# KadAMRN/Data_Free_Quantization

Hardware: AMD Instinct MI355X
Metric: weight-GB/s quantized (per-ch INT8 DFQ sweep) + top-1 delta, MobileNetV2 (higher is better)
Workload: dtype f32

## Files before the change

data_free_quantization_amd/csrc/dfq_transform.hip:

```cpp
#include "dfq_common.h"

#include <cstdlib>
#include <cstring>

#include <algorithm>
#include <chrono>
#include <cmath>
#include <mutex>
#include <new>
#include <string>
#include <vector>

namespace dfq {

static int blocks_for(int64_t n, int per_thread = 1) {
    const int64_t b = ceil_div(std::max<int64_t>(n, 1), (int64_t)kThreads * per_thread);
    return (int)std::min<int64_t>(b, 256 * 8);
}

__device__ __forceinline__ float bn_factor(float g, float v, float eps) {
    return g / sqrtf(v + eps);
}

__global__ void bn_fold_weight_kernel(float* __restrict__ w, const float* __restrict__ g,
                                      const float* __restrict__ v, float eps, int64_t rows, int64_t len) {
    const int64_t n = rows * len;
    for (int64_t i = (int64_t)blockIdx.x * blockDim.x + threadIdx.x; i < n; i += (int64_t)gridDim.x * blockDim.x) {
        const int64_t o = i / len;
        w[i] = w[i] * bn_factor(g[o], v[o], eps);
    }
}

__global__ void bn_fold_channel_kernel(float* __restrict__ bias, float* __restrict__ g, float* __restrict__ b,
                                       float* __restrict__ m, float* __restrict__ v, float* __restrict__ fake_w,
                                       float* __restrict__ fake_b, float eps, int64_t rows) {
    for (int64_t o = (int64_t)blockIdx.x * blockDim.x + threadIdx.x; o < rows; o += (int64_t)gridDim.x * blockDim.x) {
        const float go = g[o], bo = b[o], mo = m[o], vo = v[o];
        const float f = bn_factor(go, vo, eps);
        const float shift = bo - (go * mo) / sqrtf(vo + eps);
        bias[o] = bias[o] * f + shift;
        if (fake_w) fake_w[o] = fabsf(go);
        if (fake_b) fake_b[o] = bo;
        g[o] = 1.0f;
        v[o] = 1.0f;
        b[o] = 0.0f;
        m[o] = 0.0f;
    }
}

__global__ void clamp_kernel(float* __restrict__ w, int64_t n, float lo, float hi) {
    const int64_t n4 = n >> 2;
    float4* w4 = reinterpret_cast<float4*>(w);
    for (int64_t i = (int64_t)blockIdx.x * blockDim.x + threadIdx.x; i < n4; i += (int64_t)gridDim.x * blockDim.x) {
        float4 v = w4[i];
        v.x = fminf(fmaxf(v.x, lo), hi);
        v.y = fminf(fmaxf(v.y, lo), hi);
        v.z = fminf(fmaxf(v.z, lo), hi);
        v.w = fminf(fmaxf(v.w, lo), hi);
        w4[i] = v;
    }
    for (int64_t i = 4 * n4 + (int64_t)blockIdx.x * blockDim.x + threadIdx.x; i < n; i += (int64_t)gridDim.x * blockDim.x)
        w[i] = fminf(fmaxf(w[i], lo), hi);
}

__device__ __forceinline__ float absorb_c(float beta, float gamma, float n_sigma) {
    float c = beta - n_sigma * gamma;
    return (c < 0.0f) ? 0.0f : c;
}

__global__ void absorb_gemv_kernel(const float* __restrict__ w2, float* __restrict__ b2,
                                   const float* __restrict__ bn_w, const float* __restrict__ bn_b,
                                   int64_t o2, int64_t i2, int64_t khw2, int64_t o2g, float n_sigma) {
    const int lane = threadIdx.x & 63;
    const int64_t wave = (int64_t)blockIdx.x * (blockDim.x / 64) + (threadIdx.x >> 6);
    const int64_t nwaves = (int64_t)gridDim.x * (blockDim.x / 64);
    for (int64_t o = wave; o < o2; o += nwaves) {
        const int64_t g = o / o2g;
        const float* row = w2 + o * i2 * khw2;
        float acc = 0.f;
        for (int64_t i = lane; i < i2; i += 64) {
            float ssum = 0.f;
            for (int64_t k = 0; k < khw2; ++k) ssum += row[i * khw2 + k];
            const int64_t ch = g * i2 + i;
            acc += ssum * absorb_c(bn_b[ch], bn_w[ch], n_sigma);
        }
        acc = wave_sum_f(acc);
        if (lane == 0) b2[o] = b2[o] + acc;
    }
}

__global__ void absorb_channel_kernel(float* __restrict__ b1, float* __restrict__ bn_b, const float* __restrict__ bn_w,
                                      int64_t c1, float n_sigma) {
    for (int64_t c = (int64_t)blockIdx.x * blockDim.x + threadIdx.x; c < c1; c += (int64_t)gridDim.x * blockDim.x) {
        const float cc = absorb_c(bn_b[c], bn_w[c], n_sigma);
        b1[c] = b1[c] + (-cc);
        bn_b[c] = bn_b[c] + (-cc);
    }
}

__device__ __forceinline__ double ndtr_d(double a) {
    const double x = a * 0.70710678118654752440;
    const double z = fabs(x);
    if (z < 0.70710678118654752440) return 0.5 + 0.5 * erf(x);
    const double y = 0.5 * erfc(z);
    return x > 0.0 ? 1.0 - y : y;
}

__device__ __forceinline__ float bc_expect_value(float wj, float bj, int relu) {
    if (!relu) return bj;
    const float x = (-bj) / wj;
    const double xd = (double)x;
    const float pdf = (float)(exp(-(xd * xd) / 2.0) / 2.5066282746310002);
    const float cdf = (float)ndtr_d(xd);
    float ex = wj * pdf + bj * (1.0f - cdf);
    if (ex < 0.0f) ex = 0.0f;
    return ex;
}

__global__ void bc_expect_kernel(const float* __restrict__ w, const float* __restrict__ b, int64_t n, int relu,
                                 int accumulate, float* __restrict__ out) {
    for (int64_t j = (int64_t)blockIdx.x * blockDim.x + threadIdx.x; j < n; j += (int64_t)gridDim.x * blockDim.x) {
        const float ex = bc_expect_value(w[j], b[j], relu);
        out[j] = accumulate ? out[j] + ex : ex;
    }
}

__global__ void __launch_bounds__(kThreads)
bc_apply_kernel(const float* __restrict__ E, int64_t o, int64_t i2, const float* __restrict__ ex, int64_t f,
                int64_t bcols, float* __restrict__ bias, float* __restrict__ bias_vec) {
    const int lane = threadIdx.x & 63;
    const int64_t wave = (int64_t)blockIdx.x * (kThreads / 64) + (threadIdx.x >> 6);
    const int64_t nwaves = (int64_t)gridDim.x * (kThreads / 64);
    for (int64_t r = wave; r < o; r += nwaves) {
        auto get = [&](int64_t j) { return E[r * i2 + (i2 > 1 ? j : 0)] + ex[f > 1 ? j : 0]; };
        if (bias_vec)
            for (int64_t j = lane; j < bcols; j += 64) bias_vec[r * bcols + j] = get(j);
        const float sum = wave_inner_sum(get, bcols, lane);
        if (lane == 0) bias[r] = bias[r] + sum / (float)bcols;
    }
}

constexpr int64_t kBcScratch = 1024;
__global__ void __launch_bounds__(kThreads)
bc_propagate_kernel(const float* __restrict__ bias_vec, int64_t nrows, int64_t f, int threads,
                    float* __restrict__ fake_b) {
    __shared__ float scratch[kThreads / 64][kBcScratch + kBcScratch / 16];
    const int lane = threadIdx.x & 63;
    const int wv = threadIdx.x >> 6;
    float* b0s = scratch[wv];
    float* b1s = b0s + kBcScratch;
    const int64_t wave = (int64_t)blockIdx.x * (kThreads / 64) + wv;
    const int64_t nwaves = (int64_t)gridDim.x * (kThreads / 64);
    for (int64_t c = wave; c < f; c += nwaves) {
        auto get = [&](int64_t r) { return bias_vec[r * f + c]; };
        const float sum = aten_outer_col_is_cascade(nrows, f, c, threads)
                              ? wave_cascade(get, nrows, lane, b0s, b1s, kBcScratch)
                              : wave_row_sum(get, nrows, lane, b0s, b1s, kBcScratch);
        if (lane == 0) fake_b[c] = fake_b[c] + (-sum) / (float)nrows;
    }
}



constexpr int kBcMaxTerms = 8;
constexpr int64_t kBcMaxExpect = 4096;
struct BcLayerJob {
    const float* ew[kBcMaxTerms];
    const float* eb[kBcMaxTerms];
    int32_t relu[kBcMaxTerms];
    int32_t nterms;
    int32_t threads;
    float* expect_out;
    int64_t f;
    const float* E;
    int64_t o, i2, bcols;
    float* bias;
    float* vec;
    float* fake_b;
    int64_t F, nrows;
    int64_t apply_blocks;
};

constexpr int64_t kBcStage = 2048;
__global__ void __launch_bounds__(kThreads) bc_layer_kernel(BcLayerJob J) {
    __shared__ float ex[kBcMaxExpect];
    __shared__ float scratch[kThreads / 64][kBcScratch + kBcScratch / 16];
    __shared__ float stage[kThreads / 64][kBcStage];
    for (int64_t j = threadIdx.x; j < J.f; j += kThreads) {
        float v = bc_expect_value(J.ew[0][j], J.eb[0][j], J.relu[0]);
        for (int t = 1; t < J.nterms; ++t) v = v + bc_expect_value(J.ew[t][j], J.eb[t][j], J.relu[t]);
        ex[j] = v;
        if (blockIdx.x == 0) J.expect_out[j] = v;
    }
    __syncthreads();
    const int lane = threadIdx.x & 63;
    const int wv = threadIdx.x >> 6;
    const bool ebc = J.i2 > 1, xbc = J.f > 1;
    if ((int64_t)blockIdx.x < J.apply_blocks) {
        const int64_t wave = (int64_t)blockIdx.x * (kThreads / 64) + wv;
        const int64_t nwaves = J.apply_blocks * (kThreads / 64);
        float* rowv = stage[wv];
        for (int64_t r = wave; r < J.o; r += nwaves) {
            auto get = [&](int64_t j) { return J.E[r * J.i2 + (ebc ? j : 0)] + ex[xbc ? j : 0]; };
            for (int64_t j = lane; j < J.bcols; j += 64) {
                const float v = get(j);
                rowv[j] = v;
                if (J.vec) J.vec[r * J.bcols + j] = v;
            }
            wave_lds_sync();
            const float sum = wave_inner_sum([&](int64_t j) { return rowv[j]; }, J.bcols, lane);
            wave_lds_sync();
            if (lane == 0) J.bias[r] = J.bias[r] + sum / (float)J.bcols;
        }
        return;
    }
    float* b0s = scratch[wv];
    float* b1s = b0s + kBcScratch;
    const int64_t wave = ((int64_t)blockIdx.x - J.apply_blocks) * (kThreads / 64) + wv;
    const int64_t nwaves = ((int64_t)gridDim.x - J.apply_blocks) * (kThreads / 64);
    float* colv = stage[wv];
    for (int64_t c = wave; c < J.F; c += nwaves) {
        auto get = [&](int64_t r) {
            const uint32_t idx = (uint32_t)r * (uint32_t)J.F + (uint32_t)c;
            const uint32_t row = idx / (uint32_t)J.bcols, j = idx - row * (uint32_t)J.bcols;
            return J.E[(int64_t)row * J.i2 + (ebc ? j : 0)] + ex[xbc ? j : 0];
        };
        const bool cascade = aten_outer_col_is_cascade(J.nrows, J.F, c, J.threads);
        for (int64_t r = lane; r < J.nrows; r += 64) colv[r] = get(r);
        wave_lds_sync();
        auto lds = [&](int64_t r) { return colv[r]; };
        const float sum = cascade ? wave_cascade(lds, J.nrows, lane, b0s, b1s, kBcScratch)
                                  : wave_row_sum(lds, J.nrows, lane, b0s, b1s, kBcScratch);
        wave_lds_sync();
        if (lane == 0) J.fake_b[c] = J.fake_b[c] + (-sum) / (float)J.nrows;
    }
}

__device__ __forceinline__ float std_pdf(float x) {
    const double xd = (double)x;
    return (float)(exp(-(xd * xd) / 2.0) / 2.5066282746310002);
}
__device__ __forceinline__ float std_cdf(float x) { return (float)ndtr_d((double)x); }

__global__ void act_moments_kernel(const float* w_in, const float* b_in, int64_t n, int kind, int sqrt_w, float eps,
                                   int accumulate, float* mean, float* var) {
    for (int64_t j = (int64_t)blockIdx.x * blockDim.x + threadIdx.x; j < n; j += (int64_t)gridDim.x * blockDim.x) {
        const float w = sqrt_w ? sqrtf(w_in[j] + eps) : w_in[j];
        const float b = b_in[j];
        float m, v;
        if (kind == 0) {
            m = b;
            v = w * w;
        } else if (kind == 1) {
            const float x0 = (-b) / w;
            const float P0 = std_pdf(x0), C0 = std_cdf(x0);
            m = w * P0 + b * (1.0f - C0);
            const float B = ((b * b + w * w) + m * m) - (2.0f * m) * b;
            v = ((1.0f - C0) * B + (w * (b - 2.0f * m)) * P0) + (m * m) * C0;
        } else {
            const float x0 = (-b) / w, x6 = (6.0f - b) / w;
            const float P0 = std_pdf(x0), C0 = std_cdf(x0), P6 = std_pdf(x6), C6 = std_cdf(x6);
            m = (w * (P0 - P6) + b * (C6 - C0)) + 6.0f * (1.0f - C6);
            const float B = ((b * b + w * w) + m * m) - (2.0f * m) * b;
            const float d6 = 6.0f - m;
            v = ((((C6 - C0) * B + (w * -6.0f) * P6) + (w * (b - 2.0f * m)) * (P0 - P6)) + (m * m) * C0) +
                (d6 * d6) * (1.0f - C6);
        }
        if (accumulate) {
            m = mean[j] + m;
            v = var[j] + v;
        }
        mean[j] = m;
        var[j] = v;
    }
}

__global__ void act_minmax_kernel(const float* a, const float* w_in, int64_t n, int w_is_var, float eps, float nsig,
                                  float* out) {
    __shared__ float smin[4], smax[4];
    float vmin = INFINITY, vmax = -INFINITY;
    for (int64_t j = threadIdx.x; j < n; j += blockDim.x) {
        const float w = w_is_var ? sqrtf(w_in[j] + eps) : w_in[j];
        const float nw = nsig * w;
        vmin = fminf(vmin, a[j] - nw);
        vmax = fmaxf(vmax, a[j] + nw);
    }
    vmin = wave_min(vmin);
    vmax = wave_max(vmax);
    if ((threadIdx.x & 63) == 0) {
        smin[threadIdx.x >> 6] = vmin;
        smax[threadIdx.x >> 6] = vmax;
    }
    __syncthreads();
    if (threadIdx.x == 0) {
        for (int k = 1; k < (int)(blockDim.x / 64); ++k) {
            vmin = fminf(vmin, smin[k]);
            vmax = fmaxf(vmax, smax[k]);
        }
        out[0] = fminf(smin[0], vmin);
        out[1] = fmaxf(smax[0], vmax);
    }
}

__global__ void act_affine_kernel(const float* x, const float* w, const float* bias, int64_t o, int64_t i2,
                                  int64_t khw, int64_t og, float* out) {
    const int lane = threadIdx.x & 63;
    const int64_t wave = (int64_t)blockIdx.x * (blockDim.x / 64) + (threadIdx.x >> 6);
    const int64_t nwaves = (int64_t)gridDim.x * (blockDim.x / 64);
    for (int64_t r = wave; r < o; r += nwaves) {
        const int64_t g = r / og;
        float acc = 0.f;
        for (int64_t i = lane; i < i2; i += 64) {
            const float* p = w + (r * i2 + i) * khw;
            const float ws = khw == 1 ? p[0] : aten_inner_sum([&](int64_t k) { return p[k]; }, khw);
            acc += ws * x[g * i2 + i];
        }
        acc = wave_sum_f(acc);
        if (lane == 0) out[r] = bias ? acc + bias[r] : acc;
    }
}


struct BnFoldJob {
    float* w;
    float* bias;
    float* g;
    float* b;
    float* m;
    float* v;
    float* fake_w;
    float* fake_b;
    float eps;
    int32_t flags;
    int64_t rows, row_len;
    uint32_t* range_enc;
};
struct BnFoldChunk {
    int32_t job;
    int32_t pad;
    int64_t e0, e1;
};

__device__ __forceinline__ float fold_factor(const BnFoldJob& J, int64_t o) {
    const float go = ((const DFQ_GLOBAL float*)J.g)[o], ve = ((const DFQ_GLOBAL float*)J.v)[o] + J.eps;
    return (go == 1.0f && ve == 1.0f) ? 1.0f : go / sqrtf(ve);
}

__device__ __forceinline__ int64_t fold_row(const BnFoldJob& J, int64_t r0, int64_t base, float inv, int64_t i,
                                            int* rem_out) {
    const int li = (int)(i - base);
    const int len = (int)J.row_len;
    int q = (int)((float)li * inv);
    int rem = li - q * len;
    if (rem < 0) {
        --q;
        rem += len;
    } else if (rem >= len) {
        ++q;
        rem -= len;
    }
    *rem_out = rem;
    return r0 + q;
}

__device__ __forceinline__ float fold_one(const BnFoldJob& J, int64_t r0, int64_t base, float inv, int64_t i,
                                          float w) {
    int rem;
    const float f = fold_factor(J, fold_row(J, r0, base, inv, i, &rem));
    return f != 1.0f ? w * f : w;
}

__global__ void __launch_bounds__(kThreads)
bn_fold_weight_batch_kernel(const BnFoldJob* __restrict__ jobs, const BnFoldChunk* __restrict__ chunks,
                            int64_t nchunks) {
    __shared__ float smn[kThreads / kWave], smx[kThreads / kWave];
    for (int64_t c = blockIdx.x; c < nchunks; c += gridDim.x) {
        const BnFoldChunk ch = chunks[c];
        const BnFoldJob J = jobs[ch.job];
        const int64_t r0 = ch.e0 / J.row_len, base = r0 * J.row_len;
        const float inv = 1.0f / (float)J.row_len;
        float a = INFINITY, b = -INFINITY;
        const int64_t n = ch.e1 - ch.e0;
        int64_t done = 0;
        int ident = 1;
        for (int64_t r = r0 + threadIdx.x; r <= (ch.e1 - 1) / J.row_len; r += blockDim.x)
            ident &= fold_factor(J, r) == 1.0f;
        ident = __syncthreads_and(ident);
        if (ident && (reinterpret_cast<uintptr_t>(J.w + ch.e0) & 15) == 0) {
            const DFQ_GLOBAL f32x4* w4 = (const DFQ_GLOBAL f32x4*)(J.w + ch.e0);
            const int64_t n4 = n >> 2;
            for (int64_t k = threadIdx.x; k < n4; k += 4 * (int64_t)blockDim.x) {
                f32x4 v[4];
#pragma unroll
                for (int u = 0; u < 4; ++u)
                    if (k + u * (int64_t)blockDim.x < n4) v[u] = w4[k + u * blockDim.x];
#pragma unroll
                for (int u = 0; u < 4; ++u)
                    if (k + u * (int64_t)blockDim.x < n4) {
                        a = fminf(a, fminf(fminf(v[u].x, v[u].y), fminf(v[u].z, v[u].w)));
                        b = fmaxf(b, fmaxf(fmaxf(v[u].x, v[u].y), fmaxf(v[u].z, v[u].w)));
                    }
            }
            done = 4 * n4;
        } else if ((reinterpret_cast<uintptr_t>(J.w + ch.e0) & 15) == 0) {
            DFQ_GLOBAL f32x4* w4 = (DFQ_GLOBAL f32x4*)(J.w + ch.e0);
            const int64_t n4 = n >> 2;
            for (int64_t k = threadIdx.x; k < n4; k += blockDim.x) {
                const f32x4 v = w4[k];
                const int64_t i = ch.e0 + 4 * k;
                f32x4 o;
                int rem;
                const float f = fold_factor(J, fold_row(J, r0, base, inv, i, &rem));
                if (rem + 3 < (int)J.row_len) {
                    o.x = f != 1.0f ? v.x * f : v.x;
                    o.y = f != 1.0f ? v.y * f : v.y;
                    o.z = f != 1.0f ? v.z * f : v.z;
                    o.w = f != 1.0f ? v.w * f : v.w;
                } else {
                    o.x = f != 1.0f ? v.x * f : v.x;
                    o.y = fold_one(J, r0, base, inv, i + 1, v.y);
                    o.z = fold_one(J, r0, base, inv, i + 2, v.z);
                    o.w = fold_one(J, r0, base, inv, i + 3, v.w);
                }
                if (__float_as_uint(o.x) != __float_as_uint(v.x) || __float_as_uint(o.y) != __float_as_uint(v.y) ||
                    __float_as_uint(o.z) != __float_as_uint(v.z) || __float_as_uint(o.w) != __float_as_uint(v.w))
                    w4[k] = o;
                a = fminf(a, fminf(fminf(o.x, o.y), fminf(o.z, o.w)));
                b = fmaxf(b, fmaxf(fmaxf(o.x, o.y), fmaxf(o.z, o.w)));
            }
            done = 4 * n4;
        }
        DFQ_GLOBAL float* wg = (DFQ_GLOBAL float*)J.w;
        for (int64_t k = done + threadIdx.x; k < n; k += blockDim.x) {
            const int64_t i = ch.e0 + k;
            const float v = wg[i];
            const float o = fold_one(J, r0, base, inv, i, v);
            if (__float_as_uint(o) != __float_as_uint(v)) wg[i] = o;
            a = fminf(a, o);
            b = fmaxf(b, o);
        }
        if (J.range_enc) {
            a = wave_min(a);
            b = wave_max(b);
            const int lane = threadIdx.x & (kWave - 1), wv = threadIdx.x >> 6;
            if (lane == 0) {
                smn[wv] = a;
                smx[wv] = b;
            }
            __syncthreads();
            if (threadIdx.x == 0) {
                for (int k = 1; k < kThreads / kWave; ++k) {
                    a = fminf(a, smn[k]);
                    b = fmaxf(b, smx[k]);
                }
                atomicMax(&J.range_enc[0], ~enc_ord(a));
                atomicMax(&J.range_enc[1], enc_ord(b));
            }
            __syncthreads();
        }
    }
}

__global__ void bn_fold_channel_batch_kernel(const BnFoldJob* __restrict__ jobs, int32_t njobs) {
    for (int32_t j = blockIdx.x; j < njobs; j += gridDim.x) {
        const BnFoldJob J = jobs[j];
        typedef DFQ_GLOBAL float* G;
        const G g = (G)J.g, b = (G)J.b, m = (G)J.m, v = (G)J.v, bias = (G)J.bias, fw = (G)J.fake_w, fb = (G)J.fake_b;
        for (int64_t o = threadIdx.x; o < J.rows; o += blockDim.x) {
            const float go = g[o], bo = b[o], mo = m[o], vo = v[o];
            const float f = bn_factor(go, vo, J.eps);
            const float shift = bo - (go * mo) / sqrtf(vo + J.eps);
            const float b0 = (J.flags & DFQ_BN_FOLD_ZERO_BIAS) ? 0.0f : bias[o];
            bias[o] = b0 * f + shift;
            if (J.fake_w) fw[o] = fabsf(go);
            if (J.fake_b) fb[o] = bo;
            g[o] = 1.0f;
            v[o] = 1.0f;
            b[o] = 0.0f;
            m[o] = 0.0f;
        }
    }
}

__device__ __forceinline__ float qdq_nan(float x, const QParams& p, float& q) {
    const float y = qdq(x, p, q);
    return x != x ? x : y;
}

__global__ void __launch_bounds__(kThreads)
fq_given_kernel(const float* __restrict__ x, float* __restrict__ y, int64_t n, int bits, int sym, int flags,
                const float* __restrict__ min_dev, const float* __restrict__ max_dev,
                const uint32_t* __restrict__ range_enc, double gmin, double gmax, int vec4) {
    if (min_dev) gmin = (double)min_dev[0];
    if (max_dev) gmax = (double)max_dev[0];
    if (range_enc) {
        gmin = (double)dec_ord(~range_enc[0]);
        gmax = (double)dec_ord(range_enc[1]);
    }
    const QParams p = make_qparams((float)gmin, (float)gmax, bits, sym != 0, flags | DFQ_GIVEN_RANGE, gmin, gmax);
    const int64_t stride = (int64_t)gridDim.x * blockDim.x;
    float q;
    if (vec4) {
        const int64_t n4 = n >> 2;
        for (int64_t i = (int64_t)blockIdx.x * blockDim.x + threadIdx.x; i < n4; i += stride) {
            const float4 v = reinterpret_cast<const float4*>(x)[i];
            float4 o;
            o.x = qdq_nan(v.x, p, q);
            o.y = qdq_nan(v.y, p, q);
            o.z = qdq_nan(v.z, p, q);
            o.w = qdq_nan(v.w, p, q);
            reinterpret_cast<float4*>(y)[i] = o;
        }
    } else {
        for (int64_t i = (int64_t)blockIdx.x * blockDim.x + threadIdx.x; i < n; i += stride)
            y[i] = qdq_nan(x[i], p, q);
    }
}

constexpr int64_t kFqSmall = 16384;

__global__ void __launch_bounds__(kThreads)
fq_tensor_small_kernel(const float* __restrict__ x, float* __restrict__ y, int64_t n, int bits, int sym, int flags) {
    __shared__ float smn[kThreads / kWave], smx[kThreads / kWave];
    float a = INFINITY, b = -INFINITY;
    for (int64_t i = threadIdx.x; i < n; i += kThreads) {
        const float v = x[i];
        a = fminf(a, v);
        b = fmaxf(b, v);
    }
    a = wave_min(a);
    b = wave_max(b);
    const int lane = threadIdx.x & (kWave - 1), w = threadIdx.x >> 6;
    if (lane == 0) {
        smn[w] = a;
        smx[w] = b;
    }
    __syncthreads();
// ... 908 lines not shown
```

Before: 1859.

## Prefetch first bias-correction row/column into LDS during expectation compute

Before the expectation computation, each wave in the bias-correction kernel issues asynchronous global-to-LDS loads for its first row or column of E, plus an early load of the old bias value. The loads then overlap with the expectation loop and are waited on before the barrier. The first loop iteration reads the prefetched LDS values instead of global memory. This aims to hide global load latency, at the cost of more complex control flow and reliance on the global_load_lds intrinsic and its waitcnt encoding.

```diff
diff --git a/data_free_quantization_amd/csrc/dfq_transform.hip b/data_free_quantization_amd/csrc/dfq_transform.hip
--- a/data_free_quantization_amd/csrc/dfq_transform.hip
+++ b/data_free_quantization_amd/csrc/dfq_transform.hip
@@ -182,57 +182,92 @@
 };
 
 constexpr int64_t kBcStage = 2048;
+#ifndef DFQ_BC_PREFETCH
+#define DFQ_BC_PREFETCH 1
+#endif
 __global__ void __launch_bounds__(kThreads) bc_layer_kernel(BcLayerJob J) {
     __shared__ float ex[kBcMaxExpect];
     __shared__ float scratch[kThreads / 64][kBcScratch + kBcScratch / 16];
     __shared__ float stage[kThreads / 64][kBcStage];
+    const int lane = threadIdx.x & 63;
+    const int wv = wave_uniform(threadIdx.x >> 6);
+    const bool ebc = J.i2 > 1, xbc = J.f > 1;
+    const bool apply = (int64_t)blockIdx.x < J.apply_blocks;
+    const int64_t wave = ((int64_t)blockIdx.x - (apply ? 0 : J.apply_blocks)) * (kThreads / 64) + wv;
+    const int64_t nwaves = (apply ? J.apply_blocks : (int64_t)gridDim.x - J.apply_blocks) * (kThreads / 64);
+    auto gather = [&](int64_t r, int64_t c, uint32_t& j) {
+        const uint32_t idx = (uint32_t)r * (uint32_t)J.F + (uint32_t)c;
+        const uint32_t row = idx / (uint32_t)J.bcols;
+        j = idx - row * (uint32_t)J.bcols;
+        return (int64_t)row * J.i2 + (ebc ? j : 0);
+    };
+#if DFQ_BC_PREFETCH
+    float old = 0.f;
+    const bool have = wave < (apply ? J.o : J.F);
+    const int n0 = have ? (int)(apply ? J.bcols : J.nrows) : 0;
+    DFQ_LDS float* slot = (DFQ_LDS float*)stage[wv];
+    for (int k = 0; 64 * k < n0; ++k) {
+        const int e = min(lane + 64 * k, n0 - 1);
+        uint32_t j;
+        const float* src = J.E + (apply ? wave * J.i2 + (ebc ? e : 0) : gather(e, wave, j));
+        __builtin_amdgcn_global_load_lds((const DFQ_GLOBAL void*)src, (DFQ_LDS void*)(slot + 64 * k), 4, 0, 0);
+    }
+    const float* oldp = (apply ? J.bias : J.fake_b) + (have ? wave : 0);
+    if (have && lane == 0) old = *oldp;
+    bool first = true;
+#else
+    const float old = 0.f;
+    const bool first = false;
+#endif
     for (int64_t j = threadIdx.x; j < J.f; j += kThreads) {
         float v = bc_expect_value(J.ew[0][j], J.eb[0][j], J.relu[0]);
         for (int t = 1; t < J.nterms; ++t) v = v + bc_expect_value(J.ew[t][j], J.eb[t][j], J.relu[t]);
         ex[j] = v;
         if (blockIdx.x == 0) J.expect_out[j] = v;
     }
+#if DFQ_BC_PREFETCH
+    __builtin_amdgcn_s_waitcnt(0x0F70);
+#endif
     __syncthreads();
-    const int lane = threadIdx.x & 63;
-    const int wv = threadIdx.x >> 6;
-    const bool ebc = J.i2 > 1, xbc = J.f > 1;
-    if ((int64_t)blockIdx.x < J.apply_blocks) {
-        const int64_t wave = (int64_t)blockIdx.x * (kThreads / 64) + wv;
-        const int64_t nwaves = J.apply_blocks * (kThreads / 64);
+    if (apply) {
         float* rowv = stage[wv];
         for (int64_t r = wave; r < J.o; r += nwaves) {
-            auto get = [&](int64_t j) { return J.E[r * J.i2 + (ebc ? j : 0)] + ex[xbc ? j : 0]; };
             for (int64_t j = lane; j < J.bcols; j += 64) {
-                const float v = get(j);
+                const float e = first ? rowv[j] : J.E[r * J.i2 + (ebc ? j : 0)];
+                const float v = e + ex[xbc ? j : 0];
                 rowv[j] = v;
                 if (J.vec) J.vec[r * J.bcols + j] = v;
             }
             wave_lds_sync();
             const float sum = wave_inner_sum([&](int64_t j) { return rowv[j]; }, J.bcols, lane);
             wave_lds_sync();
-            if (lane == 0) J.bias[r] = J.bias[r] + sum / (float)J.bcols;
+            if (lane == 0) J.bias[r] = (first ? old : J.bias[r]) + sum / (float)J.bcols;
+#if DFQ_BC_PREFETCH
+            first = false;
+#endif
         }
         return;
     }
     float* b0s = scratch[wv];
     float* b1s = b0s + kBcScratch;
-    const int64_t wave = ((int64_t)blockIdx.x - J.apply_blocks) * (kThreads / 64) + wv;
-    const int64_t nwaves = ((int64_t)gridDim.x - J.apply_blocks) * (kThreads / 64);
     float* colv = stage[wv];
     for (int64_t c = wave; c < J.F; c += nwaves) {
-        auto get = [&](int64_t r) {
-            const uint32_t idx = (uint32_t)r * (uint32_t)J.F + (uint32_t)c;
-            const uint32_t row = idx / (uint32_t)J.bcols, j = idx - row * (uint32_t)J.bcols;
-            return J.E[(int64_t)row * J.i2 + (ebc ? j : 0)] + ex[xbc ? j : 0];
-        };
         const bool cascade = aten_outer_col_is_cascade(J.nrows, J.F, c, J.threads);
-        for (int64_t r = lane; r < J.nrows; r += 64) colv[r] = get(r);
+        for (int64_t r = lane; r < J.nrows; r += 64) {
+            uint32_t j;
+            const int64_t at = gather(r, c, j);
+            const float e = first ? colv[r] : J.E[at];
+            colv[r] = e + ex[xbc ? j : 0];
+        }
         wave_lds_sync();
         auto lds = [&](int64_t r) { return colv[r]; };
         const float sum = cascade ? wave_cascade(lds, J.nrows, lane, b0s, b1s, kBcScratch)
                                   : wave_row_sum(lds, J.nrows, lane, b0s, b1s, kBcScratch);
         wave_lds_sync();
-        if (lane == 0) J.fake_b[c] = J.fake_b[c] + (-sum) / (float)J.nrows;
+        if (lane == 0) J.fake_b[c] = (first ? old : J.fake_b[c]) + (-sum) / (float)J.nrows;
+#if DFQ_BC_PREFETCH
+        first = false;
+#endif
     }
 }
 
```

Result: no change. 1858 (-0.1%).
